# Roia2529/RayTracing-folder

Hardware: AMD Instinct MI355X
Metric: Mray/s (higher is better)
Workload: dtype f32

## Files before the change

raytracing_folder_amd/csrc/rt_kernels.hip:

```cpp
#include <hip/hip_runtime.h>
#include <math.h>
#include <string.h>
#include <stdlib.h>
#include <algorithm>
#include "rt_dev.h"

#define BIGFLOAT 1.0e30f
#define LEAF_BIT 0x80000000u
#ifndef RT_GATHER_GUESS
#define RT_GATHER_GUESS 1.2f
#endif
#ifndef RT_GATHER_RING
#define RT_GATHER_RING 128
#endif
#ifndef RT_GATHER_BAND_LO
#define RT_GATHER_BAND_LO 0.92f
#endif
#ifndef RT_GATHER_BAND_HI
#define RT_GATHER_BAND_HI 1.10f
#endif
#ifndef RT_GATHER_BATCH
#define RT_GATHER_BATCH 32
#endif
#ifndef RT_GATHER_CELL_GUESS
// ... 1403 lines not shown
__global__ __launch_bounds__(RT_BLOCK) void k_trace(DevScene S, const float *rays, long long n,
                                                    uint8_t *hit, float *z, float *p, float *N, int32_t *node, uint8_t *front)
{
    __shared__ uint32_t s_stack[RT_BVH_STACK * RT_BLOCK];
    const BvhStack stack = bvh_stack(s_stack, RT_BVH_STACK, S.bvh_spill);
    Counters cnt = {0, 0, 0, 0, 0};
    for (long long i = (long long)blockIdx.x * blockDim.x + threadIdx.x; i < n; i += (long long)gridDim.x * blockDim.x) {
        Hit h;
        h.z = BIGFLOAT; h.p = mk(0, 0, 0); h.N = mk(0, 0, 0); h.node = -1; h.front = 1;
        const bool ok = trace<false, MODEL>(S, ld3(rays + 6 * i), ld3(rays + 6 * i + 3), BIGFLOAT, h, stack, cnt);
        hit[i] = ok ? 1 : 0;
        z[i] = ok ? h.z : BIGFLOAT;
        p[3 * i] = h.p.x; p[3 * i + 1] = h.p.y; p[3 * i + 2] = h.p.z;
        N[3 * i] = h.N.x; N[3 * i + 1] = h.N.y; N[3 * i + 2] = h.N.z;
        node[i] = ok ? h.node : -1;
        front[i] = (uint8_t)h.front;
    }
}

struct Philox {
    uint32_t key0, key1, c0, c1, blk; uint32_t o0, o1, o2, o3; int used;
    __host__ __device__ void refill()
    {
        uint32_t x0 = c0, x1 = c1, x2 = blk, x3 = 0, k0 = key0, k1 = key1;
        for (int r = 0; r < 10; r++) {
            const unsigned long long p0 = (unsigned long long)0xD2511F53u * x0, p1 = (unsigned long long)0xCD9E8D57u * x2;
            const uint32_t y0 = (uint32_t)(p1 >> 32) ^ x1 ^ k0, y1 = (uint32_t)p1, y2 = (uint32_t)(p0 >> 32) ^ x3 ^ k1, y3 = (uint32_t)p0;
            x0 = y0; x1 = y1; x2 = y2; x3 = y3;
            k0 += 0x9E3779B9u; k1 += 0xBB67AE85u;
        }
        o0 = x0; o1 = x1; o2 = x2; o3 = x3;
        blk++; used = 0;
    }
    __host__ __device__ float next()
    {
        if (used >= 4) refill();
        const uint32_t v = used == 0 ? o0 : (used == 1 ? o1 : (used == 2 ? o2 : o3));
        used++;
        return (float)(v >> 8) * (1.0f / 16777216.0f);
    }
};

struct PhotonArgs {
    unsigned long long first_attempt; uint32_t n_attempts;
    uint32_t seed; int max_bounce;
    float *out;
    uint32_t *count;
    int mode;
};


__device__ bool random_photon_bounce(const rt_blinn &m, const Hit &h, V3 &rp, V3 &rd, V3 &c, Philox &rng)
{
    const V3 V = -rd;
    const V3 N = h.N;
    const float NV = dot(N, V);
    const V3 Y = NV > 0.f ? N : -N;
    float ein = 1, eout = m.ior;
    if (!h.front) { ein = m.ior; eout = 1; }
    const float eta = ein / eout;
    const V3 Z = cross(V, Y);
    const V3 X = normalize(cross(Y, Z));
    const float cosI = NV;
    const float sinI = sqrtf(fmaxf(0.0f, 1 - cosI * cosI));
    const float sinO = RMAX(0.f, RMIN(1.f, sinI * eta));
    const float cosO = sqrtf(1.f - sinO * sinO);
    const V3 tDir = (-X) * sinO - Y * cosO;
    const V3 rDir = (N * 2.f) * NV - V;
    const float C0 = (eta - 1.f) * (eta - 1.f) / ((eta + 1.f) * (eta + 1.f));
    const float rC = C0 + (1.f - C0) * powf(1.f - fabsf(cosI), 5.f);
    const float tC = 1.f - rC;
    const bool tot = (eta * sinI) > 1.001f;
    const V3 tK = ld3(m.refraction), rK = ld3(m.reflection);
    const V3 sRefr = tot ? mk(0, 0, 0) : tK * tC;
    const V3 sRefl = tot ? (rK + tK) : (rK + tK * rC);
    const V3 sDiff = ld3(m.diffuse), sSpec = ld3(m.specular);
    const float random = rng.next();
    float diffuseProb = gray(sDiff), refractionProb = gray(sRefr), reflectionProb = gray(sRefl), absorptionProb = gray(ld3(m.absorption));
    const float total = diffuseProb + reflectionProb + refractionProb + absorptionProb;
    diffuseProb /= total; refractionProb /= total; reflectionProb /= total;
    const float rcp = 1.f / total;
    const float select = random * total;
    const float luma = 0.00001f;
    int selected; float scale = 1.f;
    if (select <= refractionProb && refractionProb > luma) { selected = 0; scale = refractionProb * rcp; }
    else if (select > refractionProb && select <= refractionProb + reflectionProb && reflectionProb > luma) { selected = 1; scale = reflectionProb * rcp; }
    else if (select > refractionProb + reflectionProb && select < refractionProb + reflectionProb + diffuseProb && diffuseProb > luma) { selected = 2; scale = diffuseProb * rcp; }
    else selected = 3;
    V3 dir, BxDF;
    if (selected == 0) {
        if (m.refraction_glossiness > 0.f) {
            const float u1 = rng.next(), u2 = rng.next();
            const float r = sqrtf(1.0f - u1 * u1);
            const float phi = (float)(2 * M_PI * (double)u2);
            dir = mk(cosf(phi) * r, sinf(phi) * r, u1);
            const V3 L = normalize(dir);
            const V3 H = normalize(V + L);
            const float cosVH = RMAX(0.f, dot(V, H));
            BxDF = sRefr * powf(cosVH, m.refraction_glossiness);
        } else { dir = tDir; BxDF = sRefr; }
    } else if (selected == 1) {
        if (m.reflection_glossiness > 0.f) {
            const float u1 = rng.next(), u2 = rng.next();
            const float r = sqrtf(u1);
            const float theta = (float)(2 * M_PI * (double)u2);
            dir = mk(r * cosf(theta), r * sinf(theta), sqrtf(fmaxf(0.0f, 1 - u1)));
            const V3 L = normalize(dir);
            const V3 H = normalize(V + L);
            const float cosNH = RMAX(0.f, dot(N, H));
            BxDF = sRefl * powf(cosNH, m.reflection_glossiness);
        } else { dir = rDir; BxDF = sRefl; }
    } else if (selected == 2) {
        if (!h.front) return false;
        V3 Nt = dot(N, mk(1, 0, 0)) < 0.4f ? cross(N, mk(1, 0, 0)) : cross(N, mk(0, 0, 1));
        Nt = normalize(Nt);
        const V3 Nb = cross(N, Nt);
        const float theta = (float)((double)rng.next() * M_PI_2);
        const float phi = (float)((double)rng.next() * (2.0 * M_PI));
        dir = (Nt * cosf(phi)) * sinf(theta) + (Nb * sinf(phi)) * sinf(theta) + N * cosf(theta);
        const V3 L = normalize(dir);
        const V3 H = normalize(V + L);
        const float cosNH = RMAX(0.f, dot(N, H));
        BxDF = sDiff + sSpec * powf(cosNH, m.glossiness);
    } else return false;
    rp = h.p; rd = normalize(dir);
    c = (c * BxDF) / (1.f * scale);
    if (!h.front) c = c * attenuation(ld3(m.absorption), h.z);
    return true;
}

#define RT_PHOTON_SLOTS 8
__global__ __launch_bounds__(RT_BLOCK) void k_photon_trace(DevScene S, PhotonArgs A)
{
    __shared__ uint32_t s_stack[RT_BVH_STACK * RT_BLOCK];
    const BvhStack stack = bvh_stack(s_stack, RT_BVH_STACK, S.bvh_spill);
    Counters cnt = {0, 0, 0, 0, 0};
    const uint32_t i = blockIdx.x * blockDim.x + threadIdx.x;
    if (i >= A.n_attempts) return;
    const unsigned long long attempt = A.first_attempt + i;
    Philox rng;
    rng.key0 = A.seed; rng.key1 = 0x52544D49u; rng.c0 = (uint32_t)attempt; rng.c1 = (uint32_t)(attempt >> 32); rng.blk = 0; rng.used = 4;
    int npl = 0;
    for (int l = 0; l < S.n_lights; l++) if (S.lights[l].type == RT_LIGHT_POINT) npl++;
    uint32_t stored = 0, hits = 0;
    float *out = A.out + (size_t)i * RT_PHOTON_SLOTS * 9;
    if (npl > 0) {
        int pick = (int)(rng.next() * (float)npl);
        if (pick >= npl) pick = npl - 1;
        int li = 0;
        for (int l = 0; l < S.n_lights; l++) if (S.lights[l].type == RT_LIGHT_POINT) { if (pick == 0) { li = l; break; } pick--; }
        const rt_light &L = S.lights[li];
        V3 c = ld3(L.intensity);
        const V3 position = ld3(L.position);
        const float x = 2 * rng.next() - 1, y = 2 * rng.next() - 1, z = 2 * rng.next() - 1;
        V3 rp = position;
        V3 rd = normalize((mk(x, y, z) + position) - position);
        Hit h;
        if (A.mode == 1) {
            if (trace<false, RT_SHADE_FIN>(S, rp, rd, BIGFLOAT, h, stack, cnt)) {
                const rt_blinn *m = &S.materials[S.node_material[h.node]];
                int hitspec = gray(ld3(m->diffuse)) > 0 ? 0 : 1;
                int bounce = A.max_bounce;
                while (bounce > 0 && random_photon_bounce(*m, h, rp, rd, c, rng)) {
                    Hit nh;
                    if (!trace<false, RT_SHADE_FIN>(S, rp, rd, BIGFLOAT, nh, stack, cnt)) break;
                    m = &S.materials[S.node_material[nh.node]];
                    if (gray(ld3(m->diffuse)) > 0) {
                        if (hitspec > 1 && stored < RT_PHOTON_SLOTS) {
                            float *o = out + 9 * stored;
                            o[0] = nh.p.x; o[1] = nh.p.y; o[2] = nh.p.z; o[3] = rd.x; o[4] = rd.y; o[5] = rd.z; o[6] = c.x; o[7] = c.y; o[8] = c.z;
                            stored++;
                        }
                        hits++;
                    } else hitspec++;
                    bounce--;
                    h = nh;
                }
            }
        } else
        if (trace<false, RT_SHADE_FIN>(S, rp, rd, BIGFLOAT, h, stack, cnt)) {
            const rt_blinn *m = &S.materials[S.node_material[h.node]];
            if (gray(ld3(m->diffuse)) > 0) {
                int bounce = A.max_bounce;
                while (bounce > 0 && random_photon_bounce(*m, h, rp, rd, c, rng)) {
                    Hit nh;
                    if (!trace<false, RT_SHADE_FIN>(S, rp, rd, BIGFLOAT, nh, stack, cnt)) break;
                    m = &S.materials[S.node_material[nh.node]];
                    if (gray(ld3(m->diffuse)) > 0 && stored < RT_PHOTON_SLOTS) {
                        float *o = out + 9 * stored;
                        o[0] = nh.p.x; o[1] = nh.p.y; o[2] = nh.p.z; o[3] = rd.x; o[4] = rd.y; o[5] = rd.z; o[6] = c.x; o[7] = c.y; o[8] = c.z;
                        stored++;
                    }
                    bounce--;
                    h = nh;
                }
            }
        }
    }
    A.count[i] = stored | (hits << 16);
}

void rtk_launch_photon_trace(hipStream_t st, const DevScene &S, unsigned long long first_attempt, uint32_t n_attempts,
                             uint32_t seed, int max_bounce, float *out, uint32_t *count, int mode)
{
    PhotonArgs A; A.first_attempt = first_attempt; A.n_attempts = n_attempts; A.seed = seed; A.max_bounce = max_bounce; A.out = out; A.count = count; A.mode = mode;
    hipLaunchKernelGGL(k_photon_trace, dim3((n_attempts + RT_BLOCK - 1) / RT_BLOCK), dim3(RT_BLOCK), 0, st, S, A);
}

struct GatherArgs {
    DevPhotonMap pm;
    const float4 *qa, *qb, *qc;
    const uint32_t *count_ptr;
    uint32_t *next_batch;
    uint32_t count_cap;
    int k; float radius;
    float *sample_rgb;
    float *out_irr, *out_dir;
    int mode;
    unsigned long long *stats;
    float *cell_rk2;
    unsigned long long *fx;
};

template <int CTRL, int ROW_MASK>
__device__ __forceinline__ float dpp_f(float identity, float x)
{
    return __int_as_float(__builtin_amdgcn_update_dpp(__float_as_int(identity), __float_as_int(x), CTRL, ROW_MASK, 0xF, false));
}
template <int CTRL, int ROW_MASK>
__device__ __forceinline__ uint32_t dpp_u(uint32_t identity, uint32_t x)
{
    return (uint32_t)__builtin_amdgcn_update_dpp((int)identity, (int)x, CTRL, ROW_MASK, 0xF, false);
}
#define DPP_ROW_SHR(n) (0x110 + (n))
#define DPP_ROW_BCAST15 0x142
#define DPP_ROW_BCAST31 0x143
__device__ __forceinline__ float wave_scan_add(float x)
{
    x += dpp_f<DPP_ROW_SHR(1), 0xF>(0.0f, x); x += dpp_f<DPP_ROW_SHR(2), 0xF>(0.0f, x);
    x += dpp_f<DPP_ROW_SHR(4), 0xF>(0.0f, x); x += dpp_f<DPP_ROW_SHR(8), 0xF>(0.0f, x);
    x += dpp_f<DPP_ROW_BCAST15, 0xA>(0.0f, x); x += dpp_f<DPP_ROW_BCAST31, 0xC>(0.0f, x);
    return x;
}
__device__ __forceinline__ uint32_t wave_scan_add_u(uint32_t x)
{
    x += dpp_u<DPP_ROW_SHR(1), 0xF>(0u, x); x += dpp_u<DPP_ROW_SHR(2), 0xF>(0u, x);
    x += dpp_u<DPP_ROW_SHR(4), 0xF>(0u, x); x += dpp_u<DPP_ROW_SHR(8), 0xF>(0u, x);
    x += dpp_u<DPP_ROW_BCAST15, 0xA>(0u, x); x += dpp_u<DPP_ROW_BCAST31, 0xC>(0u, x);
    return x;
}
__device__ __forceinline__ float wave_scan_max0(float x)
{
    x = fmaxf(x, dpp_f<DPP_ROW_SHR(1), 0xF>(0.0f, x)); x = fmaxf(x, dpp_f<DPP_ROW_SHR(2), 0xF>(0.0f, x));
    x = fmaxf(x, dpp_f<DPP_ROW_SHR(4), 0xF>(0.0f, x)); x = fmaxf(x, dpp_f<DPP_ROW_SHR(8), 0xF>(0.0f, x));
    x = fmaxf(x, dpp_f<DPP_ROW_BCAST15, 0xA>(0.0f, x)); x = fmaxf(x, dpp_f<DPP_ROW_BCAST31, 0xC>(0.0f, x));
    return x;
}
__device__ __forceinline__ float wave_sum(float x) { return __int_as_float(__builtin_amdgcn_readlane(__float_as_int(wave_scan_add(x)), 63)); }
__device__ __forceinline__ uint32_t wave_sum_u(uint32_t x) { return (uint32_t)__builtin_amdgcn_readlane((int)wave_scan_add_u(x), 63); }
__device__ __forceinline__ float wave_max0(float x) { return __int_as_float(__builtin_amdgcn_readlane(__float_as_int(wave_scan_max0(x)), 63)); }

__device__ __forceinline__ void fold32(float a, float b, float &ab)
{
    const auto r = __builtin_amdgcn_permlane32_swap(__float_as_uint(a), __float_as_uint(b), false, false);
    ab = __uint_as_float(r[0]) + __uint_as_float(r[1]);
}
__device__ __forceinline__ void fold16(float x, float y, float &xy)
{
    const auto r = __builtin_amdgcn_permlane16_swap(__float_as_uint(x), __float_as_uint(y), false, false);
    xy = __uint_as_float(r[0]) + __uint_as_float(r[1]);
}
__device__ __forceinline__ float row_total(float x)
{
    x += dpp_f<DPP_ROW_SHR(8), 0xF>(0.0f, x); x += dpp_f<DPP_ROW_SHR(4), 0xF>(0.0f, x);
    x += dpp_f<DPP_ROW_SHR(2), 0xF>(0.0f, x); x += dpp_f<DPP_ROW_SHR(1), 0xF>(0.0f, x);
    return x;
}
__device__ __forceinline__ void wave_sum6(float v0, float v1, float v2, float v3, float v4, float v5, float out[6])
{
    float s01, s23, s45, t0123, t45;
    fold32(v0, v1, s01); fold32(v2, v3, s23); fold32(v4, v5, s45);
    fold16(s01, s23, t0123);
    fold16(s45, s45, t45);
    t0123 = row_total(t0123); t45 = row_total(t45);
    out[0] = __int_as_float(__builtin_amdgcn_readlane(__float_as_int(t0123), 15));
    out[2] = __int_as_float(__builtin_amdgcn_readlane(__float_as_int(t0123), 31));
    out[1] = __int_as_float(__builtin_amdgcn_readlane(__float_as_int(t0123), 47));
    out[3] = __int_as_float(__builtin_amdgcn_readlane(__float_as_int(t0123), 63));
    out[4] = __int_as_float(__builtin_amdgcn_readlane(__float_as_int(t45), 15));
    out[5] = __int_as_float(__builtin_amdgcn_readlane(__float_as_int(t45), 47));
}

__device__ __forceinline__ float lane_f(float v, int l) { return __int_as_float(__builtin_amdgcn_readlane(__float_as_int(v), l)); }
__device__ __forceinline__ uint32_t lane_u(uint32_t v, int l) { return (uint32_t)__builtin_amdgcn_readlane((int)v, l); }

__device__ __forceinline__ float box_dist2(const float4 *b, float px, float py, float pz)
{
    RT_FP_CONTRACT
    const float4 lo = b[0], hi = b[1];
    const float dx = fmaxf(fmaxf(lo.x - px, px - hi.x), 0.0f);
    const float dy = fmaxf(fmaxf(lo.y - py, py - hi.y), 0.0f);
    const float dz = fmaxf(fmaxf(lo.z - pz, pz - hi.z), 0.0f);
    return dx * dx + dy * dy + dz * dz;
}

__device__ __forceinline__ void wave_sync()
{
    __builtin_amdgcn_fence(__ATOMIC_RELEASE, "wavefront");
    __builtin_amdgcn_wave_barrier();
    __builtin_amdgcn_fence(__ATOMIC_ACQUIRE, "wavefront");
}

struct GatherLds {
    uint16_t leaves[RT_GATHER_BATCH][RT_LEAFLIST_CAP];
    uint32_t subs[RT_SUBLIST_CAP + RT_SUBS_PER_STEP];
    union alignas(16) {
        uint32_t hist[256];
        struct { float sel_d[64]; uint32_t sel_i[64]; uint32_t sel_n; };
    };
    float4   ring_a[RT_GATHER_RING];
    float2   ring_b[RT_GATHER_RING];
};

__device__ __forceinline__ float byte_over_255(uint32_t c)
{
    const float r_hi = 0x1.010102p-8f, r_lo = -0x1.fdfdfep-33f;
    const float x = (float)c;
    return __fmaf_rn(x, r_hi, x * r_lo);
}

struct Cand { float d2; float4 pa, pb; };
struct GatherQuery { float px, py, pz, nx, ny, nz, rq2, kscale; };
__device__ __forceinline__ Cand make_cand(float4 pa, float4 pb, const GatherQuery &Q)
{
    RT_FP_CONTRACT
    Cand c;
    c.pa = pa; c.pb = pb;
    const float dfx = pa.x - Q.px, dfy = pa.y - Q.py, dfz = pa.z - Q.pz;
    const float d2 = dfx * dfx + dfy * dfy + dfz * dfz;
    const bool away = (pa.w * Q.nx + pb.x * Q.ny + pb.y * Q.nz) >= 0;
    c.d2 = away ? __builtin_inff() : d2;
    return c;
}
__device__ __forceinline__ uint32_t cand_key(const Cand &c, const GatherQuery &Q) { return (uint32_t)(c.d2 * Q.kscale); }

template <class F>
__device__ __forceinline__ void scan_subleaves(const DevPhotonMap &pm, const uint32_t *ids, uint32_t n_sub, int lane,
                                               const GatherQuery &Q, F &&f)
{
    if (n_sub == 0) return;
    const uint32_t n_iter = (n_sub + RT_SUBS_PER_STEP - 1u) / RT_SUBS_PER_STEP;
    const uint32_t *mine = ids + (uint32_t)lane / RT_SUB_PHOTONS;
    const uint32_t lane_off = ((uint32_t)lane % RT_SUB_PHOTONS) * 16u;
    const char *pa = (const char *)pm.pa, *pb = (const char *)pm.pb;
    auto ld = [&](uint32_t it, float4 &a, float4 &b, uint32_t &slot) {
        const uint32_t off = (mine[RT_SUBS_PER_STEP * it] * (RT_SUB_PHOTONS * 16u)) | lane_off;
        slot = off;
        a = *(const float4 *)(pa + off);
        b = *(const float4 *)(pb + off);
    };
    float4 a0, b0, a1, b1;
    uint32_t s0, s1;
    ld(0u, a0, b0, s0);
    uint32_t it = 0;
    for (; it + 1 < n_iter; it += 2) {
        ld(it + 1, a1, b1, s1);
        f(make_cand(a0, b0, Q), s0);
        ld(min(it + 2, n_iter - 1), a0, b0, s0);
        f(make_cand(a1, b1, Q), s1);
    }
    if (it < n_iter) f(make_cand(a0, b0, Q), s0);
}

#ifndef RT_GATHER_WAVES_PER_EU
#define RT_GATHER_WAVES_PER_EU 5
#endif
template <bool FX = false>
__attribute__((amdgpu_waves_per_eu(RT_GATHER_WAVES_PER_EU, RT_GATHER_WAVES_PER_EU)))
__global__ __launch_bounds__(64 * RT_GATHER_WAVES) void k_gather(GatherArgs G)
{
    __shared__ GatherLds lds_all[RT_GATHER_WAVES];
    GatherLds &L = lds_all[threadIdx.x >> 6];
    const int lane = threadIdx.x & 63;
    uint32_t nq = *G.count_ptr;
    if (nq > G.count_cap) nq = G.count_cap;
    if (nq == 0) return;
    const uint32_t n_leaves = G.pm.n_leaves;
    const uint32_t n_sub_total = n_leaves * RT_LEAF_SUBS;
    const float r2 = G.radius * G.radius;
    const uint32_t K = (uint32_t)G.k;
    unsigned long long visited = 0;
    uint32_t n_rounds = 0, n_slow = 0, n_reads = 0;
    float pred_rk2 = 0.0f;

    const uint32_t n_batches = (nq + (uint32_t)RT_GATHER_BATCH - 1u) / (uint32_t)RT_GATHER_BATCH;
    const float guess_c = RT_GATHER_GUESS * (float)K * G.pm.cell * G.pm.cell / (float)M_PI;

    uint32_t xcc;
    asm volatile("s_getreg_b32 %0, hwreg(HW_REG_XCC_ID)" : "=s"(xcc));
    xcc &= 7u;
    const uint32_t seg_len = (n_batches + 7u) / 8u;
    uint32_t seg = xcc;
    for (;;) {
        const uint32_t seg_first = seg * seg_len;
        const uint32_t seg_size = seg_first >= n_batches ? 0u : min(seg_len, n_batches - seg_first);
        uint32_t got = 0;
        if (lane == 0) got = atomicAdd(G.next_batch + seg * RT_CTR_STRIDE, 1u);
        got = (uint32_t)__builtin_amdgcn_readfirstlane((int)got);
        if (got >= seg_size) {
            uint32_t *const done_mask = G.next_batch + 8 * RT_CTR_STRIDE;
            uint32_t done = 0;
            if (lane == 0) {
                done = __hip_atomic_load(done_mask, __ATOMIC_RELAXED, __HIP_MEMORY_SCOPE_AGENT);
                if (!((done >> seg) & 1u)) atomicOr(done_mask, 1u << seg);
            }
            done = ((uint32_t)__builtin_amdgcn_readfirstlane((int)done) | (1u << seg)) & 255u;
            if (done == 255u) break;
            const uint32_t rot = ((done ^ 255u) | ((done ^ 255u) << 8)) >> (seg + 1u);
            seg = (seg + 1u + ((uint32_t)__ffs((int)rot) - 1u)) & 7u;
            continue;
        }
        const uint32_t qbase = (seg_first + got) * (uint32_t)RT_GATHER_BATCH;
        const uint32_t qi = qbase + lane;
        const bool have = lane < RT_GATHER_BATCH && qi < nq;
        float4 a = make_float4(0, 0, 0, 0), b = make_float4(0, 0, 0, 0), c = make_float4(0, 0, 0, 0);
        if (have) { a = G.qa[qi]; b = G.qb[qi]; c = G.qc[qi]; }
        bool pending = have;
        float f_pr = 0, f_pg = 0, f_pb = 0, f_dx = 0, f_dy = 0, f_dz = 0, f_area = -1.0f;
        bool finish = false;
        float r2cur = r2;
        float cell_pred = 0.0f;
        uint32_t cell_index = 0;
        uint32_t walk_start = 1;
        if (have && n_leaves > 1) {
            const float fx = (a.x - G.pm.grid_min[0]) * G.pm.inv_cell, fy = (a.y - G.pm.grid_min[1]) * G.pm.inv_cell, fz = (a.z - G.pm.grid_min[2]) * G.pm.inv_cell;
            const int gx = min(max((int)fx, 0), G.pm.grid_dim[0] - 1);
            const int gy = min(max((int)fy, 0), G.pm.grid_dim[1] - 1);
            const int gz = min(max((int)fz, 0), G.pm.grid_dim[2] - 1);
            cell_index = (uint32_t)(((size_t)gz * G.pm.grid_dim[1] + gy) * G.pm.grid_dim[0] + gx);
            const bool in_grid = fx >= 0.0f && fy >= 0.0f && fz >= 0.0f && (int)fx == gx && (int)fy == gy && (int)fz == gz;
            if (G.pm.cell_start && in_grid && G.radius <= G.pm.start_radius) walk_start = G.pm.cell_start[cell_index];
            const uint32_t cnt = G.pm.grid[cell_index];
            r2cur = fminf(fmaxf(guess_c / (float)(cnt > 0u ? cnt : 1u), r2 * 1.0e-4f), r2);
            if (G.cell_rk2) {
                cell_pred = G.cell_rk2[cell_index];
                if (cell_pred > 0.0f) r2cur = fminf(fmaxf(cell_pred * RT_GATHER_CELL_GUESS, r2 * 1.0e-4f), r2);
                else if (cell_pred < 0.0f) r2cur = r2;
            }
        }

        while (ballot64(pending)) {
            static_assert(RT_GATHER_BATCH == 32, "phase A pairs lane l with lane l + 32");
            const bool upper = lane >= 32;
            auto from_lower = [](float v) { return __uint_as_float(__builtin_amdgcn_permlane32_swap(__float_as_uint(v), __float_as_uint(v), false, false)[0]); };
            const float wx = from_lower(a.x), wy = from_lower(a.y), wz = from_lower(a.z), wr2 = from_lower(r2cur);
            const uint32_t wstart = __builtin_amdgcn_permlane32_swap(walk_start, walk_start, false, false)[0];
            const bool walking = ((uint32_t)ballot64(pending) >> (lane & 31)) & 1u;
            auto both_halves = [](uint32_t mine, int bits) {
                const auto r = __builtin_amdgcn_permlane32_swap(mine, mine, false, false);
                return r[0] | (r[1] << bits);
            };
            uint32_t nl = 0;
            auto list_leaf = [&](uint32_t leaf) {
                if (!upper && nl < RT_LEAFLIST_CAP) L.leaves[lane][nl] = (uint16_t)leaf;
                nl++;
            };
            if (walking && n_leaves) {
                if (box_dist2(G.pm.tbox + 2, wx, wy, wz) < wr2) {
                    if (n_leaves == 1) list_leaf(0u);
                    else {
                        uint32_t node = wstart;
                        uint32_t pd = (31u - (uint32_t)__clz((int)node)) >> 1;
                        uint32_t todo_mask = 0;
                        for (;;) {
                            if (4u * node < 2u * n_leaves && 2u * node < n_leaves) {
                                const float4 *gb = G.pm.tbox + 8 * (size_t)node + (upper ? 4 : 0);
                                uint32_t m2 = 0;
                                if (box_dist2(gb, wx, wy, wz) < wr2) m2 |= 1u;
                                if (box_dist2(gb + 2, wx, wy, wz) < wr2) m2 |= 2u;
                                const uint32_t m4 = both_halves(m2, 2);
                                if (4u * node >= n_leaves) {
                                    for (int i = 0; i < 4; i++) if ((m4 >> i) & 1u) list_leaf(4u * node + (uint32_t)i - n_leaves);
                                } else if (m4) {
                                    const uint32_t i = (uint32_t)__ffs((int)m4) - 1u;
                                    todo_mask |= (m4 & ~(1u << i)) << (4u * pd);
                                    node = 4u * node + i; pd++;
                                    continue;
                                }
                            } else {
                                const float4 *cb = G.pm.tbox + 4 * (size_t)node + (upper ? 2 : 0);
                                const uint32_t m2 = both_halves(box_dist2(cb, wx, wy, wz) < wr2 ? 1u : 0u, 1);
                                if (m2 & 1u) list_leaf(2u * node - n_leaves);
                                if (m2 & 2u) list_leaf(2u * node + 1u - n_leaves);
                            }
                            if (!todo_mask) break;
                            const uint32_t bit = 31u - (uint32_t)__clz((int)todo_mask);
                            const uint32_t d = bit >> 2;
                            const uint32_t nib = (todo_mask >> (4u * d)) & 15u;
                            const uint32_t i = (uint32_t)__ffs((int)nib) - 1u;
                            todo_mask &= ~(1u << (4u * d + i));
                            node = ((node >> (2u * (pd - d))) << 2) + i;
                            pd = d + 1u;
                        }
                    }
                }
            }
            wave_sync();
            unsigned long long todo = ballot64(pending);
            while (todo) {
                const int q = __ffsll((long long)todo) - 1;
                todo &= todo - 1;
                GatherQuery Q;
                Q.px = lane_f(a.x, q); Q.py = lane_f(a.y, q); Q.pz = lane_f(a.z, q);
                Q.nx = lane_f(a.w, q); Q.ny = lane_f(b.x, q); Q.nz = lane_f(b.y, q);
                Q.rq2 = lane_f(r2cur, q);
                Q.kscale = 16777000.0f / Q.rq2;
                const float rq2 = Q.rq2;
                const uint32_t qnl = lane_u(nl, q);
                const bool final_round = rq2 >= r2;
                const bool slow = qnl > RT_LEAFLIST_CAP;
                const uint32_t dummy_sub = n_sub_total;
                uint32_t n_sub = 0;
                wave_sync();
                if (!slow) {
                    for (uint32_t base = 0; base < qnl * RT_LEAF_SUBS; base += 64u) {
                        const uint32_t e = base + (uint32_t)lane;
                        const bool have_e = (e / RT_LEAF_SUBS) < qnl;
                        const uint32_t sub = have_e ? (uint32_t)L.leaves[q][e / RT_LEAF_SUBS] * RT_LEAF_SUBS + (e % RT_LEAF_SUBS) : 0u;
                        const float bd = have_e ? box_dist2(G.pm.sbox + 2 * (size_t)sub, Q.px, Q.py, Q.pz) : __builtin_inff();
                        const unsigned long long m = ballot64(bd < rq2);
                        if (bd < rq2) L.subs[n_sub + lanes_below(m)] = sub;
                        n_sub += (uint32_t)__popcll(m);
                    }
                    if (lane < RT_SUBS_PER_STEP) L.subs[n_sub + lane] = dummy_sub;
                    wave_sync();
                } else {
                    for (uint32_t base = 0; base < n_sub_total; base += 64u) {
                        const uint32_t sub = base + (uint32_t)lane;
                        const float bd = sub < n_sub_total ? box_dist2(G.pm.sbox + 2 * (size_t)sub, Q.px, Q.py, Q.pz) : __builtin_inff();
                        n_sub += (uint32_t)__popcll(ballot64(bd < rq2));
                    }
                }
                n_rounds++; n_slow += slow ? 1u : 0u; n_reads += n_sub;
                auto for_each = [&](auto &&f) {
                    if (!slow) { scan_subleaves(G.pm, L.subs, n_sub, lane, Q, f); return; }
                    for (uint32_t base = 0; base < n_sub_total; base += 64u) {
                        const uint32_t sub = base + (uint32_t)lane;
                        const float bd = sub < n_sub_total ? box_dist2(G.pm.sbox + 2 * (size_t)sub, Q.px, Q.py, Q.pz) : __builtin_inff();
                        const unsigned long long m = ballot64(bd < rq2);
                        if (!m) continue;
                        wave_sync();
                        if (bd < rq2) L.subs[lanes_below(m)] = sub;
                        const uint32_t cnt = (uint32_t)__popcll(m);
                        if (lane < RT_SUBS_PER_STEP) L.subs[cnt + lane] = dummy_sub;
                        wave_sync();
                        scan_subleaves(G.pm, L.subs, cnt, lane, Q, f);
                    }
                };
                float s_pr = 0, s_pg = 0, s_pb = 0, s_dx = 0, s_dy = 0, s_dz = 0;
                auto accumulate5 = [&](float dirx, float diry, float dirz, float maxp, uint32_t cbits, bool take) {
                    RT_FP_CONTRACT
                    if (!take) return;
                    const float mp = take ? maxp : 0.0f;
                    s_pr += byte_over_255(cbits & 255u) * mp; s_pg += byte_over_255((cbits >> 8) & 255u) * mp; s_pb += byte_over_255((cbits >> 16) & 255u) * mp;
                    s_dx += dirx * mp; s_dy += diry * mp; s_dz += dirz * mp;
                };
                auto accumulate = [&](const float4 &pa, const float4 &pb, bool take) { accumulate5(pa.w, pb.x, pb.y, pb.z, __float_as_uint(pb.w), take); };

                uint32_t M = 0;
                float area_d2 = rq2;
                bool done_plain = false;
                if (final_round && lane_f(cell_pred, q) < 0.0f) {
                    for_each([&](const Cand &cd, uint32_t) {
                        M += (uint32_t)__popcll(ballot64(cd.d2 < rq2));
                        accumulate(cd.pa, cd.pb, cd.d2 < rq2);
                    });
                    visited += n_sub;
                    if (M <= K) done_plain = true;
                    else { M = 0; s_pr = s_pg = s_pb = s_dx = s_dy = s_dz = 0; n_reads += n_sub; }
                }
                if (!done_plain) {
                *(uint4 *)&L.hist[4 * lane] = make_uint4(0u, 0u, 0u, 0u);
                wave_sync();
                const float kscale_bin = Q.kscale * (1.0f / 65536.0f);
                { const float cp = lane_f(cell_pred, q); if (cp > 0.0f) pred_rk2 = cp; }
                const float pk = (pred_rk2 > 0.0f && pred_rk2 < rq2) ? pred_rk2 : rq2 * (1.0f / RT_GATHER_GUESS);
                const float t_lo = RT_GATHER_BAND_LO * pk;
                const float t_hi = final_round ? rq2 : fminf(RT_GATHER_BAND_HI * pk, rq2);
                uint32_t n_ring = 0;
                for_each([&](const Cand &cd, uint32_t) {
                    const unsigned long long m_ok = ballot64(cd.d2 < rq2);
                    const unsigned long long m_lo = ballot64(cd.d2 < t_lo);
                    const unsigned long long mr = ballot64(cd.d2 < t_hi) & ~m_lo;
                    M += (uint32_t)__popcll(m_ok);
                    if (cd.d2 < rq2) atomicAdd(&L.hist[(uint32_t)(cd.d2 * kscale_bin)], 1u);
                    accumulate(cd.pa, cd.pb, cd.d2 < t_lo);
                    if (mr) {
                        if (cd.d2 < t_hi && !(cd.d2 < t_lo)) {
                            const uint32_t at = n_ring + lanes_below(mr);
                            if (at < (uint32_t)RT_GATHER_RING) {
                                L.ring_a[at] = make_float4(cd.d2, cd.pa.w, cd.pb.x, cd.pb.y);
                                L.ring_b[at] = make_float2(cd.pb.z, cd.pb.w);
                            }
                        }
                        n_ring += (uint32_t)__popcll(mr);
                    }
                });
                visited += n_sub;
                if (!final_round && M <= K) {
                    float grow = 1.5f * (float)K / (float)(M > 0 ? M : 1u);
                    grow = fminf(fmaxf(grow, 2.0f), 16.0f);
                    if (lane == q) r2cur = fminf(rq2 * grow, r2);
                    continue;
                }
                area_d2 = rq2;
                if (M > K) {
                    uint32_t need = K;
                    uint32_t prefix = 0;
                    int shift = 16;
                    uint32_t in_bin = 0;
                    for (;;) {
                        wave_sync();
                        const uint4 h4 = *(const uint4 *)&L.hist[4 * lane];
                        const uint32_t h0 = h4.x, h1 = h4.y, h2 = h4.z, h3 = h4.w;
                        const uint32_t mine = h0 + h1 + h2 + h3;
                        const uint32_t incl = wave_scan_add_u(mine);
                        const uint32_t excl = incl - mine;
                        const unsigned long long m = ballot64(incl >= need);
                        const int owner = __ffsll((long long)m) - 1;
                        uint32_t digit = 0, before = 0, cntb = 0;
                        if (lane == owner) {
                            const uint32_t cum = excl;
                            if (cum + h0 >= need) { digit = 4 * lane; before = cum; cntb = h0; }
                            else if (cum + h0 + h1 >= need) { digit = 4 * lane + 1; before = cum + h0; cntb = h1; }
                            else if (cum + h0 + h1 + h2 >= need) { digit = 4 * lane + 2; before = cum + h0 + h1; cntb = h2; }
                            else { digit = 4 * lane + 3; before = cum + h0 + h1 + h2; cntb = h3; }
                        }
                        digit = lane_u(digit, owner); before = lane_u(before, owner); cntb = lane_u(cntb, owner);
                        need -= before;
                        prefix |= digit << shift;
                        in_bin = cntb;
                        if (in_bin <= 64u || shift == 0) break;
                        shift -= 8;
                        wave_sync();
                        *(uint4 *)&L.hist[4 * lane] = make_uint4(0u, 0u, 0u, 0u);
                        wave_sync();
                        const uint32_t hi_mask = ~((1u << (shift + 8)) - 1u) & 0xFFFFFFu;
                        for_each([&](const Cand &cd, uint32_t) {
                            const uint32_t key = cand_key(cd, Q);
                            if (cd.d2 < rq2 && (key & hi_mask) == prefix) atomicAdd(&L.hist[(key >> shift) & 255u], 1u);
                        });
                    }
                    const uint32_t bin_mask = ~((1u << shift) - 1u) & 0xFFFFFFu;
                    wave_sync();
                    if (lane == 0) L.sel_n = 0;
                    wave_sync();
                    uint32_t tie_taken = 0;
                    float tmax = 0.0f;
                    bool from_ring = false;
                    {
                        const uint32_t bin_lo = (uint32_t)(t_lo * Q.kscale) >> 16, bin_hi = (uint32_t)(t_hi * Q.kscale) >> 16;
                        const uint32_t kbin = prefix >> 16;
                        from_ring = shift == 16 && in_bin <= 64u && n_ring <= (uint32_t)RT_GATHER_RING && bin_lo < kbin && (t_hi >= rq2 || kbin < bin_hi);
                    }
                    if (from_ring) {
                        for (uint32_t base = 0; base < n_ring; base += 64u) {
                            const uint32_t idx = base + (uint32_t)lane;
                            const bool have = idx < n_ring;
                            const float4 ra = have ? L.ring_a[idx] : make_float4(3.0e38f, 0, 0, 0);
                            const float2 rb = have ? L.ring_b[idx] : make_float2(0, 0);
                            const uint32_t kb = (uint32_t)(ra.x * Q.kscale) & bin_mask;
                            const bool take = have && kb < prefix;
                            const bool inb = have && kb == prefix;
                            const unsigned long long mb = ballot64(inb);
                            if (mb) {
                                const uint32_t sbase = lane_u(L.sel_n, 0);
                                if (inb) {
                                    const uint32_t at = sbase + lanes_below(mb);
                                    if (at < 64u) { L.sel_d[at] = ra.x; L.sel_i[at] = idx; }
                                }
                                wave_sync();
                                if (lane == 0) L.sel_n = sbase + (uint32_t)__popcll(mb);
                                wave_sync();
                            }
                            accumulate5(ra.y, ra.z, ra.w, rb.x, __float_as_uint(rb.y), take);
                        }
                    }
                    if (!from_ring) {
                    n_reads += n_sub;
                    s_pr = s_pg = s_pb = s_dx = s_dy = s_dz = 0;
                    for_each([&](const Cand &cd, uint32_t s) {
                        const bool ok = cd.d2 < rq2;
                        const uint32_t kb = cand_key(cd, Q) & bin_mask;
                        bool take = ok && kb < prefix;
                        const bool inb = ok && kb == prefix;
                        const unsigned long long mb = ballot64(inb);
                        if (in_bin <= 64u) {
                            if (mb) {
                                uint32_t base = 0;
                                const int leader = __ffsll((long long)mb) - 1;
                                if (lane == leader) { base = L.sel_n; L.sel_n = base + (uint32_t)__popcll(mb); }
                                base = lane_u(base, leader);
                                if (inb) {
                                    const uint32_t at = base + lanes_below(mb);
                                    if (at < 64u) { L.sel_d[at] = cd.d2; L.sel_i[at] = s; }
                                }
                            }
                        } else {
                            const uint32_t rank = tie_taken + lanes_below(mb);
                            if (inb && rank < need) { take = true; tmax = fmaxf(tmax, cd.d2); }
                            tie_taken += (uint32_t)__popcll(mb);
                        }
                        accumulate(cd.pa, cd.pb, take);
                    });
                    }
                    wave_sync();
                    if (in_bin <= 64u) {
                        const uint32_t n_sel = lane_u(min(L.sel_n, 64u), 0);
                        const bool mine = (uint32_t)lane < n_sel;
                        const float md = mine ? L.sel_d[lane] : 3.0e38f;
                        uint32_t rank = 0;
                        for (uint32_t j = 0; j < n_sel; j++) {
                            const float od = L.sel_d[j];
                            rank += (od < md || (od == md && j < (uint32_t)lane)) ? 1u : 0u;
                        }
                        if (mine && rank < need) {
                            const uint32_t si = L.sel_i[lane];
                            if (from_ring) {
                                const float4 ra = L.ring_a[si];
                                const float2 rb = L.ring_b[si];
                                accumulate5(ra.y, ra.z, ra.w, rb.x, __float_as_uint(rb.y), true);
                            } else
                                accumulate(*(const float4 *)((const char *)G.pm.pa + si), *(const float4 *)((const char *)G.pm.pb + si), true);
                            tmax = md;
                        }
                    }
                    area_d2 = wave_max0(tmax);
                    pred_rk2 = area_d2;
                }
                else if (M > 0) {
                    if (n_ring <= (uint32_t)RT_GATHER_RING) {
                        for (uint32_t base = 0; base < n_ring; base += 64u) {
                            const uint32_t idx = base + (uint32_t)lane;
                            if (idx < n_ring) {
                                const float4 ra = L.ring_a[idx];
                                const float2 rb = L.ring_b[idx];
                                accumulate5(ra.y, ra.z, ra.w, rb.x, __float_as_uint(rb.y), true);
                            }
                        }
                    } else {
                        n_reads += n_sub;
                        s_pr = s_pg = s_pb = s_dx = s_dy = s_dz = 0;
                        for_each([&](const Cand &cd, uint32_t) { accumulate(cd.pa, cd.pb, cd.d2 < rq2); });
                    }
                }
                }
                {
                    float t[6];
                    wave_sum6(s_pr, s_pg, s_pb, s_dx, s_dy, s_dz, t);
                    if (lane == q) {
                        f_pr = t[0]; f_pg = t[1]; f_pb = t[2]; f_dx = t[3]; f_dy = t[4]; f_dz = t[5];
                        f_area = M > 0 ? area_d2 : -1.0f;
                        finish = true;
                        pending = false;
                    }
                }
            }
            if (finish) {
                float irr_r = f_pr, irr_g = f_pg, irr_b = f_pb, dx = f_dx, dy = f_dy, dz = f_dz;
                if (G.cell_rk2 && n_leaves > 1) {
                    if (f_area > 0.0f && f_area < r2) G.cell_rk2[cell_index] = f_area;
                    else if (r2cur >= r2) G.cell_rk2[cell_index] = -1.0f;
                }
                if (f_area >= 0.0f) {
                    const float area = (float)M_PI * f_area;
                    if (area > 0) { const float inv = 1.0f / area; irr_r *= inv; irr_g *= inv; irr_b *= inv; }
                    const float l = sqrtf(dx * dx + dy * dy + dz * dz);
                    dx /= l; dy /= l; dz /= l;
                }
                if (G.mode == 1) {
                    const size_t qq = (size_t)qi;
                    G.out_irr[3 * qq] = irr_r; G.out_irr[3 * qq + 1] = irr_g; G.out_irr[3 * qq + 2] = irr_b;
                    G.out_dir[3 * qq] = dx; G.out_dir[3 * qq + 1] = dy; G.out_dir[3 * qq + 2] = dz;
                } else {
                    const float nx = a.w, ny = b.x, nz = b.y, wr = b.z, wg = b.w, wb = c.x;
                    const uint32_t slot = __float_as_uint(c.y);
                    float theta = nx * (-dx) + ny * (-dy) + nz * (-dz);
                    theta = theta > 0.0f ? theta : 0.0f;
                    if constexpr (FX) fx_add(G.fx + 3 * (size_t)slot, (wr * irr_r) * theta, (wg * irr_g) * theta, (wb * irr_b) * theta);
                    else {
                        float *dst = G.sample_rgb + 3 * (size_t)slot;
                        atomicAdd(dst, (wr * irr_r) * theta);
                        atomicAdd(dst + 1, (wg * irr_g) * theta);
                        atomicAdd(dst + 2, (wb * irr_b) * theta);
                    }
                }
                finish = false;
            }
            wave_sync();
        }
    }
    if (G.stats) {
        __shared__ unsigned long long s_acc[4];
        if (threadIdx.x < 4) s_acc[threadIdx.x] = 0;
        __syncthreads();
        if (lane == 0 && visited) {
            atomicAdd(&s_acc[0], visited * (unsigned long long)RT_SUB_PHOTONS);
            atomicAdd(&s_acc[1], (unsigned long long)n_rounds);
            atomicAdd(&s_acc[2], (unsigned long long)n_slow);
            atomicAdd(&s_acc[3], (unsigned long long)n_reads * RT_SUB_PHOTONS / 32ull);
        }
        __syncthreads();
        if (threadIdx.x < 4) {
            const int slot = threadIdx.x == 0 ? ST_PHOTONS_VISITED : threadIdx.x == 1 ? ST_GATHER_ROUNDS : threadIdx.x == 2 ? ST_GATHER_SLOW : ST_GATHER_LEAF_READS;
            const unsigned long long x = s_acc[threadIdx.x];
            if (x) atomicAdd(&G.stats[ST_AT(slot)], x);
        }
    }
    if (G.stats && blockIdx.x == 0 && threadIdx.x == 0) atomicAdd(&G.stats[ST_AT(ST_PHOTON_QUERIES)], (unsigned long long)nq);
}

struct ResolveArgs {
    DevCamera cam; DevTiles tiles;
    uint32_t q0, npix;
    int min_sample, max_sample;
    float threshold; float inv_gamma;
    int phase;
    float bg[3];
    DevScene S;
    uint8_t *rgb8; float *z; uint8_t *count;
    uint2 *packed;
    int direct_mode;
};

__device__ __forceinline__ uint8_t float_to_byte(float r)
{
    const float s = r * 255;
    if (!(s == s)) return 0;
    if (s <= -2147483648.0f) return 0;
    if (s >= 2147483647.0f) return 255;
    const int v = (int)s;
    return (uint8_t)(v < 0 ? 0 : (v > 255 ? 255 : v));
}

#ifndef RT_RESOLVE_TILE
#define RT_RESOLVE_TILE 8
#endif
__global__ __launch_bounds__(256) void k_resolve(DevWork W, ResolveArgs A)
{
    __shared__ float s_tile[4][64 * (3 * RT_RESOLVE_TILE + 1)];
    float *tile = s_tile[threadIdx.x >> 6];
    const int lane = threadIdx.x & 63;
    const uint32_t npix = A.phase == 1 ? W.counts[CNT_PIXLIST] : A.npix;
    const uint32_t npix_round = (npix + 63u) & ~63u;
    if (blockIdx.x == 0 && threadIdx.x == 0 && W.stats) {
        uint32_t pr = 0;
        for (int l = 1; l < CNT_PHOTONQ; l++) pr = max(pr, W.counts[l]);
        atomicMax(&W.stats[ST_AT(ST_PEAK_RAYS)], (unsigned long long)pr);
        atomicMax(&W.stats[ST_AT(ST_PEAK_QUERIES)], (unsigned long long)max(W.counts[CNT_PHOTONQ], W.counts[CNT_CAUSTICQ]));
    }
    for (uint32_t i = blockIdx.x * blockDim.x + threadIdx.x; i < npix_round; i += gridDim.x * blockDim.x) {
        const uint32_t i0 = i - (uint32_t)lane;
        const bool staged = A.phase == 0 && i0 + 64u <= npix;
        const bool in_range = i < npix;
        const uint32_t ql = in_range ? (A.phase == 1 ? W.pixel_list[i] : i) : 0u;
        int x = 0, y = 0;
        const bool valid = in_range && pixel_of(A.tiles, A.cam, A.q0 + ql, x, y);
        if (A.packed && in_range && !valid && A.phase == 0) A.packed[(size_t)A.q0 + ql] = make_uint2(0u, 0u);
        if (!staged && !valid) continue;
        const size_t index = (size_t)y * A.cam.width + x;
        const float *rgb = W.sample_rgb + 3 * (size_t)ql * A.max_sample;
        const uint8_t *hitf = W.sample_hit + (size_t)ql * A.max_sample;
        const float *zs = W.sample_z + (size_t)ql * A.max_sample;
        const int ns = A.phase == 1 ? A.max_sample : A.min_sample;
        const bool packed_hits = (A.max_sample & 15) == 0;
        const int nblk = (ns + 63) >> 6;
        auto block_mask = [&](int b) -> unsigned long long {
            const int base = 64 * b, cnt = min(64, ns - base);
            unsigned long long m = 0;
            if (packed_hits) {
                const uint4 *h4 = (const uint4 *)(hitf + base);
                for (int t = 0; 16 * t < cnt; t++) {
                    const uint4 w = h4[t];
                    const uint32_t b16 = (((w.x & 0x01010101u) * 0x01020408u) >> 24) | ((((w.y & 0x01010101u) * 0x01020408u) >> 24) << 4) |
                                         ((((w.z & 0x01010101u) * 0x01020408u) >> 24) << 8) | ((((w.w & 0x01010101u) * 0x01020408u) >> 24) << 12);
                    m |= (unsigned long long)(b16 & 0xFFFFu) << (16 * t);
                }
            } else {
                for (int j = 0; j < cnt; j++) if (hitf[base + j]) m |= 1ull << j;
            }
            if (cnt < 64) m &= (1ull << cnt) - 1ull;
            return m;
        };
        int n = 0, last = -1;
        for (int b = 0; b < nblk; b++) { const unsigned long long m = block_mask(b); n += __popcll(m); if (m) last = 64 * b + 63 - __clzll((long long)m); }
        float hitz = 0;
        if (last >= 0) hitz = zs[last];
        auto for_hit_samples = [&](auto &&visit) {
            const float *wave_rgb = W.sample_rgb + 3 * (size_t)i0 * A.max_sample;
            for (int b = 0; b < nblk; b++) {
                const unsigned long long hm = block_mask(b);
                const int base = 64 * b, cnt = min(64, ns - base);
                if (staged) {
                    for (int t0 = 0; t0 < cnt; t0 += RT_RESOLVE_TILE) {
                        const int tn = min(RT_RESOLVE_TILE, cnt - t0);
                        const int run = 3 * tn;
                        __builtin_amdgcn_wave_barrier();
                        for (int k = lane; k < 64 * run; k += 64) {
                            const int pix = k / run, off = k - pix * run;
                            tile[pix * (3 * RT_RESOLVE_TILE + 1) + off] = wave_rgb[(size_t)pix * 3 * A.max_sample + 3 * (base + t0) + off];
                        }
                        __builtin_amdgcn_fence(__ATOMIC_RELEASE, "workgroup");
                        __builtin_amdgcn_wave_barrier();
                        __builtin_amdgcn_fence(__ATOMIC_ACQUIRE, "workgroup");
                        const float *mine = tile + lane * (3 * RT_RESOLVE_TILE + 1);
                        for (int j = 0; j < tn; j++) if ((hm >> (t0 + j)) & 1ull) visit(mine[3 * j], mine[3 * j + 1], mine[3 * j + 2]);
                    }
                } else {
                    for (int j = 0; j < cnt; j++) if ((hm >> j) & 1ull) visit(rgb[3 * (base + j)], rgb[3 * (base + j) + 1], rgb[3 * (base + j) + 2]);
                }
            }
        };
        bool over = false;
        if (A.phase == 0 && A.min_sample != A.max_sample && (staged || n > 0)) {
            const float ninverse = (float)(1.0 / (n > 0 ? n : 1));
            float sum[3] = {0, 0, 0}, sq[3] = {0, 0, 0};
            for_hit_samples([&](float r, float g, float b) {
                const float t3[3] = {r, g, b};
                for (int c = 0; c < 3; c++) {
                    sum[c] += t3[c];
                    sq[c] = (float)((double)sq[c] + (double)t3[c] * (double)t3[c]);
                }
            });
            for (int c = 0; c < 3; c++) {
                const float avg = ninverse * sum[c];
                const float var = (float)((double)(sq[c] * ninverse) + (double)avg * (double)avg - (double)(2 * avg * ninverse * sum[c]));
                if (var > A.threshold) over = true;
            }
            over = over && n > 0 && valid;
            if (over) W.pixel_list[atomicAdd(&W.counts[CNT_PIXLIST], 1u)] = ql;
        }
        float c0 = 0, c1 = 0, c2 = 0;
        if (staged || n > 0) {
            const float inv = 1 / (float)(n > 0 ? n : 1);
            for_hit_samples([&](float r, float g, float b) { c0 += r * inv; c1 += g * inv; c2 += b * inv; });
        }
        if (!valid || over) continue;
        float g[3];
        uint8_t cnt_byte = 0;
        float zval = BIGFLOAT;
        if (n > 0) {
            g[0] = powf(c0, A.inv_gamma); g[1] = powf(c1, A.inv_gamma); g[2] = powf(c2, A.inv_gamma);
            cnt_byte = (n <= A.min_sample) ? 0 : 255;
            zval = hitz;
        } else {
            const V3 bgc = textured_color(A.S, ld3(A.bg), A.S.bg_map, mk((float)x / A.cam.width, (float)y / A.cam.height, 0));
            g[0] = powf(bgc.x, A.inv_gamma); g[1] = powf(bgc.y, A.inv_gamma); g[2] = powf(bgc.z, A.inv_gamma);
        }
        const uint32_t r8 = float_to_byte(g[0]), g8 = float_to_byte(g[1]), b8 = float_to_byte(g[2]);
        if (A.packed) {
            const uint32_t zb = __float_as_uint(zval);
            A.packed[(size_t)A.q0 + ql] = make_uint2(r8 | (g8 << 8) | (b8 << 16) | (zb << 24), (zb >> 8) | ((uint32_t)cnt_byte << 24));
        } else {
            A.count[index] = cnt_byte;
            A.z[index] = zval;
            A.rgb8[3 * index] = (uint8_t)r8; A.rgb8[3 * index + 1] = (uint8_t)g8; A.rgb8[3 * index + 2] = (uint8_t)b8;
        }
    }
}

static inline int grid_for(unsigned long long work, int block, int max_blocks)
{
    unsigned long long b = (work + block - 1) / block;
    if (b < 1) b = 1;
    if (b > (unsigned long long)max_blocks) b = max_blocks;
    return (int)b;
}

static SlotMap make_slotmap(const DevCamera &cam, const DevTiles &tiles_prepared, uint32_t q0, int max_sample, int mode)
{
    SlotMap m; m.tiles = tiles_prepared; m.width = cam.width; m.height = cam.height; m.q0 = q0; m.max_sample = max_sample; m.mode = mode;
    m.div_ms = fastdiv_make((uint32_t)(max_sample > 0 ? max_sample : 1));
    return m;
}
static uint32_t wf_lds_rays()
{
    const char *e = getenv("RT_WF_LDS_RAYS");
    const long v = e ? atol(e) : 0;
    return v > 0 ? (uint32_t)v : 0u;
}
static bool wavefront_usable(const DevScene &S, const rt_params &P, bool tex)
{
    static int wavefront = -1;
    if (wavefront < 0) { const char *e = getenv("RT_TRACER"); wavefront = (e && !strcmp(e, "levels")) ? 0 : 1; }
    static int p12 = -1;
    if (p12 < 0) { const char *e = getenv("RT_P12_TRACER"); p12 = (e && !strcmp(e, "levels")) ? 0 : 1; }
    const bool model_ok = P.shade_model == RT_SHADE_FIN || P.shade_model == RT_SHADE_P13 || (P.shade_model == RT_SHADE_P12 && p12 && P.hemisphere_sample <= 2);
    if (!wavefront || !model_ok) return false;
    return S.max_bvh_depth <= (tex ? WfCfg<true>::BVH : WfCfg<false>::BVH) + (S.max_bvh_depth > RT_BVH_LDS ? RT_BVH_SPILL : 0);
}

bool rtk_wavefront_usable(const DevScene &S, const rt_params &P)
{
    return wavefront_usable(S, P, S.material_maps != nullptr || S.env_map.texture != RT_MAP_NONE);
}

template <int MODEL>
static void launch_wavefront_model(hipStream_t st, bool tex, bool fx, int wgrid, const ShadeCtx &C, const PrimaryArgs &A)
{
    if (fx) {
        if (tex) hipLaunchKernelGGL((k_wavefront<MODEL, true, true>), dim3(wgrid), dim3(RT_BLOCK), 0, st, C, A);
        else hipLaunchKernelGGL((k_wavefront<MODEL, false, true>), dim3(wgrid), dim3(RT_BLOCK), 0, st, C, A);
    } else {
        if (tex) hipLaunchKernelGGL((k_wavefront<MODEL, true>), dim3(wgrid), dim3(RT_BLOCK), 0, st, C, A);
        else hipLaunchKernelGGL((k_wavefront<MODEL, false>), dim3(wgrid), dim3(RT_BLOCK), 0, st, C, A);
    }
}
static void launch_wavefront(hipStream_t st, int model, bool tex, bool fx, int wgrid, const ShadeCtx &C, const PrimaryArgs &A)
{
    if (model == RT_SHADE_FIN) launch_wavefront_model<RT_SHADE_FIN>(st, tex, fx, wgrid, C, A);
    else if (model == RT_SHADE_P12) launch_wavefront_model<RT_SHADE_P12>(st, tex, fx, wgrid, C, A);
    else launch_wavefront_model<RT_SHADE_P13>(st, tex, fx, wgrid, C, A);
}

void rtk_launch_primary(hipStream_t st, const DevScene &S, const DevWork &W, const rt_params &P,
                        const DevRayQueue &qout, uint32_t *qout_count, const DevCamera &cam,
                        const DevTiles &tiles, uint32_t q0, uint32_t npix, int j0, int ns,
                        int max_sample, int mode, const float *rays, int max_blocks, unsigned long long *fx)
{
    ShadeCtx C; C.S = S; C.S.bvh_spill = W.bvh_spill; C.W = W; C.P = P; C.qout = qout; C.qout_count = qout_count; C.fx = fx;
    PrimaryArgs A; A.cam = cam; A.tiles = tiles; A.q0 = q0; A.npix = npix; A.j0 = j0; A.ns = ns;
    A.max_sample = max_sample; A.mode = mode; A.rays = rays; A.lds_rays = wf_lds_rays();
    tiles_prepare(A.tiles);
    A.div_ns = fastdiv_make((uint32_t)(ns > 0 ? ns : 1));
    const int grid = grid_for((unsigned long long)npix * ns, RT_BLOCK, max_blocks);
    const bool tex = S.material_maps != nullptr || S.env_map.texture != RT_MAP_NONE;
    C.lds_a = C.lds_b = C.lds_c = nullptr; C.lds_count = nullptr; C.lds_cap = 0;
    C.sm = make_slotmap(cam, A.tiles, q0, max_sample, mode);
    if (wavefront_usable(S, P, tex)) {
        const int wgrid = grid_for((unsigned long long)npix * ns, RT_BLOCK, 256 * (tex ? RT_WF_TEX_WAVES : RT_WF_WAVES));
        launch_wavefront(st, P.shade_model, tex, fx != nullptr, wgrid, C, A);
        return;
    }
#define RT_LAUNCH_PRIMARY(M) do { if (fx) { if (tex) hipLaunchKernelGGL((k_primary<M, true, true>), dim3(grid), dim3(RT_BLOCK), 0, st, C, A); \
                                            else hipLaunchKernelGGL((k_primary<M, false, true>), dim3(grid), dim3(RT_BLOCK), 0, st, C, A); } \
                                  else if (tex) hipLaunchKernelGGL((k_primary<M, true>), dim3(grid), dim3(RT_BLOCK), 0, st, C, A); \
                                  else hipLaunchKernelGGL((k_primary<M, false>), dim3(grid), dim3(RT_BLOCK), 0, st, C, A); } while (0)
    switch (P.shade_model) {
    case RT_SHADE_P13: RT_LAUNCH_PRIMARY(RT_SHADE_P13); break;
    case RT_SHADE_P12: RT_LAUNCH_PRIMARY(RT_SHADE_P12); break;
    case RT_SHADE_P6: RT_LAUNCH_PRIMARY(RT_SHADE_P6); break;
    case RT_SHADE_P3: RT_LAUNCH_PRIMARY(RT_SHADE_P3); break;
    default: RT_LAUNCH_PRIMARY(RT_SHADE_FIN);
    }
#undef RT_LAUNCH_PRIMARY
}
// ... 121 lines not shown
```

Baseline: 9211.

## Prune subleaves to distance shell and reuse partial sums in gather rescans

Adds a near/far box-distance test that compacts the subleaf list to those whose distance range overlaps the band still undecided, between the already-summed radius t_lo and the selection bin or the query radius. The rescan then keeps its existing partial sums instead of zeroing them, and adds or subtracts contributions by sign so photons already counted below t_lo are not re-accumulated. This is meant to cut the memory reads and work of the second selection pass. It adds an extra compaction pass with wave syncs, and correctness now depends on epsilon-padded shell bounds and the signed-correction trick.

```diff
diff --git a/raytracing_folder_amd/csrc/rt_kernels.hip b/raytracing_folder_amd/csrc/rt_kernels.hip
--- a/raytracing_folder_amd/csrc/rt_kernels.hip
+++ b/raytracing_folder_amd/csrc/rt_kernels.hip
@@ -1729,6 +1729,17 @@
     const float dy = fmaxf(fmaxf(lo.y - py, py - hi.y), 0.0f);
     const float dz = fmaxf(fmaxf(lo.z - pz, pz - hi.z), 0.0f);
     return dx * dx + dy * dy + dz * dz;
+}
+
+__device__ __forceinline__ void box_near_far2(const float4 *b, float px, float py, float pz, float &near2, float &far2)
+{
+    RT_FP_CONTRACT
+    const float4 lo = b[0], hi = b[1];
+    const float ax = lo.x - px, bx = px - hi.x, ay = lo.y - py, by = py - hi.y, az = lo.z - pz, bz = pz - hi.z;
+    const float dx = fmaxf(fmaxf(ax, bx), 0.0f), dy = fmaxf(fmaxf(ay, by), 0.0f), dz = fmaxf(fmaxf(az, bz), 0.0f);
+    const float ex = fmaxf(fabsf(ax), fabsf(bx)), ey = fmaxf(fabsf(ay), fabsf(by)), ez = fmaxf(fabsf(az), fabsf(bz));
+    near2 = dx * dx + dy * dy + dz * dz;
+    far2 = ex * ex + ey * ey + ez * ez;
 }
 
 __device__ __forceinline__ void wave_sync()
@@ -1969,6 +1980,29 @@
                     }
                 }
                 n_rounds++; n_slow += slow ? 1u : 0u; n_reads += n_sub;
+                auto keep_shell = [&](float lo, float hi) {
+                    if (slow) return;
+                    uint32_t out = 0;
+                    for (uint32_t base = 0; base < n_sub; base += 64u) {
+                        const uint32_t j = base + (uint32_t)lane;
+                        uint32_t id = 0;
+                        bool keep = false;
+                        if (j < n_sub) {
+                            float near2, far2;
+                            id = L.subs[j];
+                            box_near_far2(G.pm.sbox + 2 * (size_t)id, Q.px, Q.py, Q.pz, near2, far2);
+                            keep = far2 * (1.0f + 0x1p-10f) >= lo && near2 * (1.0f - 0x1p-10f) < hi;
+                        }
+                        const unsigned long long m = ballot64(keep);
+                        wave_sync();
+                        if (keep) L.subs[out + lanes_below(m)] = id;
+                        out += (uint32_t)__popcll(m);
+                    }
+                    wave_sync();
+                    if (lane < RT_SUBS_PER_STEP) L.subs[out + lane] = dummy_sub;
+                    wave_sync();
+                    n_sub = out;
+                };
                 auto for_each = [&](auto &&f) {
                     if (!slow) { scan_subleaves(G.pm, L.subs, n_sub, lane, Q, f); return; }
                     for (uint32_t base = 0; base < n_sub_total; base += 64u) {
@@ -2114,8 +2148,11 @@
                         }
                     }
                     if (!from_ring) {
+                    {
+                        const float bin_d2_lo = (float)prefix / Q.kscale, bin_d2_hi = (float)(prefix + (1u << shift)) / Q.kscale;
+                        keep_shell(fminf(t_lo, bin_d2_lo) * (1.0f - 0x1p-10f), fmaxf(t_lo, bin_d2_hi) * (1.0f + 0x1p-10f));
+                    }
                     n_reads += n_sub;
-                    s_pr = s_pg = s_pb = s_dx = s_dy = s_dz = 0;
                     for_each([&](const Cand &cd, uint32_t s) {
                         const bool ok = cd.d2 < rq2;
                         const uint32_t kb = cand_key(cd, Q) & bin_mask;
@@ -2138,7 +2175,8 @@
                             if (inb && rank < need) { take = true; tmax = fmaxf(tmax, cd.d2); }
                             tie_taken += (uint32_t)__popcll(mb);
                         }
-                        accumulate(cd.pa, cd.pb, take);
+                        const bool summed = cd.d2 < t_lo;
+                        accumulate5(cd.pa.w, cd.pb.x, cd.pb.y, take ? cd.pb.z : -cd.pb.z, __float_as_uint(cd.pb.w), take != summed);
                     });
                     }
                     wave_sync();
@@ -2176,9 +2214,9 @@
                             }
                         }
                     } else {
+                        keep_shell(t_lo * (1.0f - 0x1p-10f), __builtin_inff());
                         n_reads += n_sub;
-                        s_pr = s_pg = s_pb = s_dx = s_dy = s_dz = 0;
-                        for_each([&](const Cand &cd, uint32_t) { accumulate(cd.pa, cd.pb, cd.d2 < rq2); });
+                        for_each([&](const Cand &cd, uint32_t) { accumulate(cd.pa, cd.pb, cd.d2 < rq2 && !(cd.d2 < t_lo)); });
                     }
                 }
                 }
```

After: 9291, median of 6. No clear change (+0.9%).
